# bcosm/CantorRL

Hardware: AMD Instinct MI355X
Metric: env-steps/sec (batched episodes) (higher is better)
Workload: dtype f64+f32; 1 GPU; configs[1]: 65,536 parallel envs/GPU, European call (BS rolling-ATM marks), GBM, v2 env, train_ppo_v2 reward; config_index=2, envs_per_gpu=65536, episode_length=252, mode=rollout, rollout_k=256, action_sets=1, parallelism=env-shard x1

## Files before the change

### cantorrl_amd/csrc/he_math.h

```cpp
#pragma once

#include <hip/hip_runtime.h>
#include <stdint.h>

#define HE_HD __host__ __device__ __forceinline__

namespace he {

HE_HD double fma_k(double a, double b, double c) {
#if defined(__HIP_DEVICE_COMPILE__)
    double r;
    asm("v_fma_f64 %0, %1, %2, %3" : "=v"(r) : "v"(a), "v"(b), "s"(c));
    return r;
#else
    return fma(a, b, c);
#endif
}

HE_HD double fma_kb(double a, double k, double c) {
#if defined(__HIP_DEVICE_COMPILE__)
    double r;
    asm("v_fma_f64 %0, %1, %2, %3" : "=v"(r) : "v"(a), "s"(k), "v"(c));
    return r;
#else
// ... 87 lines not shown
}

HE_HD float div_int_byf(float a, float b, float y) {
    const float q = a * y;
    return fmaf(fmaf(-q, b, a), y, q);
}
HE_HD double div_int_by(double a, double b, double y) {
    const double q = a * y;
    return fma(fma(-q, b, a), y, q);
}

HE_HD float div_f32_by(float a, double b, double y64) {
    const double ad = (double)a;
    const double q = ad * y64;
    const double r = fma(-q, b, ad);
    const float res = (float)fma(r, y64, q);
    return (a == 0.0f || !(fabsf(a) <= 3.4028234663852886e38f)) ? (float)q : res;
}

HE_HD float div_f32_byf(float a, float b, float y) {
    const float q = a * y;
    const float res = fmaf(fmaf(-q, b, a), y, q);
    return (a == 0.0f || !(fabsf(a) <= 3.4028234663852886e38f)) ? q : res;
}

HE_HD int32_t trade_round(float f, int32_t mt) {
    const float r = rintf(f);
    const bool ok = fabsf(r) < 9.2233720368547758e18f;
    const float lo = -(float)mt, hi = (float)mt;
#if defined(__HIP_DEVICE_COMPILE__)
    return ok ? (int32_t)__builtin_amdgcn_fmed3f(r, lo, hi) : -mt;
#else
    const float c = r < lo ? lo : (r > hi ? hi : r);
    const int32_t v = ok ? (int32_t)c : 0;
    return ok ? v : -mt;
#endif
}

HE_HD uint32_t episode_wrap_le(uint32_t t, uint32_t k, uint32_t T) {
    const uint32_t s = t + k;
    return s >= T ? s - T : s;
}
HE_HD uint32_t episode_wrap(uint32_t t, uint32_t k, uint32_t T) {
    return k <= T ? episode_wrap_le(t, k, T) : (t + k) % T;
}

// ... 564 lines not shown
```

### cantorrl_amd/csrc/hedge_env.hip

```cpp
#include <hip/hip_runtime.h>
#include <hip/hip_ext.h>

#include <math.h>
#include <stdarg.h>
#include <stdio.h>
#include <stdlib.h>
#include <string.h>

#include <chrono>
#include <new>
#include <type_traits>

#include "vn_moments.h"
#include <string>
#include <vector>

#include "../../include/hedge_env.h"
#include "he_math.h"

using namespace he;

namespace {

#define GLOBAL __attribute__((address_space(1)))
// ... 61 lines not shown
    float s0s_f, inv_s0s_f;
    double s0s_d, inv_s0s_d;
    double inv_252;
    float init_cash_f;
    double tcpc, slip_frac, lam, w, theta, initial_cash;
    double shares_d, inv_shares;
    float shares_f;
    int32_t shares_zero;
    float r_f, tenor_f;
    double r_d, tenor_d, sqrt_tenor;
    int32_t tenor_small;
    uint32_t key0, key1;
    double s0;
    double var;
    float var_f;
    double sqrt_var, drift, sqrt_dt, mu, dt;
    BSConst bs;
    int32_t mark;
    double fe_K;
    float g_sigma, g_num_drift;
    double g_sst;
    double g_inv_sst;
    float g_sst_f, g_inv_sst_f;
    float sqrt_tenor_f;
    double h_kappa, h_theta, h_xi, h_rho, h_sqrt1mrho2;
    int32_t den_const;
    double den, inv_den;
    int32_t M;
    float4* tileA;
    float4* tileB;
    float rstv[4 + kObs];
    const float4* rec;
    const float4* recg;
    int64_t n_paths;
    int64_t rstride;
    int32_t roff;
    int32_t book_n;
    const BookOpt* book;
    const double* book_tab;
    int32_t book_rows;
    double bk_sig, bk_isig, bk_s2, bk_lam;
    double book_rst;
    double* tileC;
#ifdef HE_TIMING
    uint64_t* tim;
#endif
// ... 122 lines not shown
            cd = (S > K) ? 1.0 : ((S == K) ? 0.5 : 0.0);
            pd = (S < K) ? -1.0 : ((S == K) ? -0.5 : 0.0);
            gam = 0.0;
        } else {
            float Kc = np_maxf(K, 1e-6f);
            float num = logf(S / Kc) + num_drift;
            double d1;
            if (sst < 1e-9) {
                float sg = (num > 0.0f) ? 1.0f : ((num < 0.0f) ? -1.0f : num);
                d1 = (double)(sg * 10.0f);
            } else {
                d1 = CONST_VAR ? (double)num * p.g_inv_sst : (double)num / sst;
            }
            double n1 = ndtr(d1);
            cd = n1;
            pd = n1 - 1.0;
            double gd = (double)S * sst;
            gam = (fabs(gd) < 1e-9) ? 0.0 : norm_pdf(d1) / gd;
        }
    }
    return make_float4((float)cd, (float)gam, (float)pd, 0.0f);
}

__device__ __forceinline__ float ncdf_tail(float d1, float ph) {
    const float a = fminf(fabsf(d1), 14.0f);
    const float w = 2.0f * __builtin_amdgcn_rcpf(a + 2.0f);
    float r = -2.690903097e-02f;
    r = fmaf(r, w, 6.361111253e-02f);
    r = fmaf(r, w, 2.313483953e-01f);
    r = fmaf(r, w, -1.219161630e+00f);
    r = fmaf(r, w, 2.182162046e+00f);
    r = fmaf(r, w, -1.785471797e+00f);
    r = fmaf(r, w, 4.304344356e-01f);
    r = fmaf(r, w, -1.690988056e-02f);
    r = fmaf(r, w, 3.958457112e-01f);
    r = fmaf(r, w, 4.983069301e-01f);
    r = fmaf(r, w, 5.000579357e-01f);
    return ph * (r * w);
}

template <bool CONST_VAR>
__device__ __forceinline__ float4 greeks_fast(const Params& p, float S, float v) {
    float cd, gam, pd;
    const float K = rintf(S);
    if (S <= 1e-6f) {
        cd = (K == 0.0f) ? 0.5f : ((K > 0.0f) ? 0.0f : 1.0f);
        pd = (K == 0.0f) ? -0.5f : ((K < 0.0f) ? 0.0f : -1.0f);
        gam = 0.0f;
// ... 28 lines not shown
            const float ph = expf(-0.5f * (d1 * d1)) * 0.398942280401432678f;
            const float tail = ncdf_tail(d1, ph);
            cd = (d1 >= 0.0f) ? 1.0f - tail : tail;
            pd = (d1 >= 0.0f) ? -tail : tail - 1.0f;
            const float gd = S * sstf;
            gam = (fabsf(gd) < 1e-9f) ? 0.0f : ph * __builtin_amdgcn_rcpf(gd);
        }
    }
    return make_float4(cd, gam, pd, 0.0f);
}

__device__ __forceinline__ float4 replay_greeks(const Params& p, float S, float v) {
    return greeks<false>(p, S, v);
}

__device__ __forceinline__ float div_f32_core(float a, float b) {
    float r = __builtin_amdgcn_rcpf(b);
    r = fmaf(fmaf(-b, r, 1.0f), r, r);
    float q = a * r;
    q = fmaf(fmaf(-b, q, a), r, q);
    return fmaf(fmaf(-b, q, a), r, q);
}

__device__ __forceinline__ float logf_normal(float x) {
    const float r = __builtin_amdgcn_logf(x);
    const float hi = r * 0x1.62e42ep-1f;
    float t = fmaf(r, 0x1.62e42ep-1f, -hi);
    t = fmaf(r, 0x1.efa39ep-25f, t);
    return (fabsf(r) < __builtin_inff()) ? hi + t : r;
}
__device__ __forceinline__ float expf_nonpos(float x) {
    const float hi = x * 0x1.715476p+0f;
    float t = fmaf(x, 0x1.715476p+0f, -hi);
    const float k = rintf(hi);
    t = fmaf(x, 0x1.4ae0bep-26f, t);
    const float e = __builtin_amdgcn_exp2f((hi - k) + t);
    const float v = ldexpf(e, (int)k);
    return (x >= -0x1.9d1da0p+6f || x != x) ? v : 0.0f;
}

__device__ __forceinline__ float4 greeks_lean(float S, float num_drift, float inv_sst_f, float sstf) {
    const float K = rintf(S);
    const float Kc = np_maxf(K, 1e-6f);
    const float num = logf_normal(div_f32_core(S, Kc)) + num_drift;
    const float d1 = num * inv_sst_f;
    const float ph = expf_nonpos(-0.5f * (d1 * d1)) * 0.398942280401432678f;
    const float tail = ncdf_tail(d1, ph);
    float cd = (d1 >= 0.0f) ? 1.0f - tail : tail;
    float pd = (d1 >= 0.0f) ? -tail : tail - 1.0f;
    const float gd = S * sstf;
    float ge = ph * __builtin_amdgcn_rcpf(gd);
    float ct = (K == 0.0f) ? 0.5f : ((K > 0.0f) ? 0.0f : 1.0f);
    float pt = (K == 0.0f) ? -0.5f : ((K < 0.0f) ? 0.0f : -1.0f);
    HE_OPAQUE3(ge, ct, pt);
    float gam = (fabsf(gd) < 1e-9f) ? 0.0f : ge;
    const bool tiny = S <= 1e-6f;
    cd = tiny ? ct : cd;
    pd = tiny ? pt : pd;
    gam = tiny ? 0.0f : gam;
    return make_float4(cd, gam, pd, 0.0f);
}

__device__ __forceinline__ int32_t clamp_pos(int32_t n, int32_t maxh) {
    int32_t r;
    asm("v_med3_i32 %0, %1, %2, %3" : "=v"(r) : "v"(n), "v"(-maxh), "v"(maxh));
    return r;
}

__device__ __forceinline__ float lag_return(float S, float Sp) {
    float q = (S - Sp) / Sp;
    HE_OPAQUE1(q);
    return (Sp == 0.0f) ? 0.0f : np_clipf(q, -1.0f, 1.0f);
}

__device__ __forceinline__ float lag_return_lean(float S, float Sp) {
    const float d = S - Sp;
    float q = div_f32_core((d > Sp) ? Sp : d, Sp);
    HE_OPAQUE1(q);
    return (Sp == 0.0f) ? 0.0f : np_clipf(q, -1.0f, 1.0f);
}

template <bool FAST = false, bool EP = false>
__device__ __forceinline__ void make_obs(const Params& p, const Env& e, const Mkt& m, float4 g, float Sp,
                                         float vp, float* o) {
    if (EP) {
        o[0] = div_f32_by(m.S, e.s0s_d, e.inv_s0s_d);
        o[1] = div_f32_by(m.C, e.s0s_d, e.inv_s0s_d);
        o[2] = div_f32_by(m.P, e.s0s_d, e.inv_s0s_d);
    } else if (FAST || p.s0s_const) {
        o[0] = div_f32_by(m.S, p.s0s_d, p.inv_s0s_d);
        o[1] = div_f32_by(m.C, p.s0s_d, p.inv_s0s_d);
        o[2] = div_f32_by(m.P, p.s0s_d, p.inv_s0s_d);
    } else {
        float s0s = np_maxf(e.s0, 25.0f);
        o[0] = m.S / s0s;
        o[1] = m.C / s0s;
        o[2] = m.P / s0s;
    }
    if (FAST || p.maxh != 0) {
// ... 1288 lines not shown
    static constexpr int prod = lanes;
    static constexpr int penvs = kLdsEnvs / lanes;
    static constexpr int threads = 64 * (2 + prod);
    static constexpr int H = kLdsM / lanes;
    static constexpr int minwaves = (BOOK || HESTON) ? kLdsMinWavesBook
                                                     : (HE_LDS_BALANCE ? 4 : (4 * (2 + prod) + 3) / 4 + 1);
    static_assert(H * lanes == kLdsM && penvs * lanes == kLdsEnvs, "producer lane layout");
};

constexpr int kLdsBookRows = 256;
constexpr int lds_thp_rows() { return 512; }
template <int MODE, bool BOOK, bool LEAN = false>
struct LdsMarketT {
    static constexpr int NB = 2;
    static constexpr bool THP = LEAN && !BOOK;
    double thp[THP ? lds_thp_rows() : 1];
    float2 sc[NB][kLdsM][kLdsEnvs];
    float pp[NB][kLdsM][kLdsEnvs];
    float stage[2][kLdsEnvs * kObs];
    double bk[BOOK ? 2 : 1][BOOK ? kLdsM : 1][kLdsEnvs];
    float vv[MODE == HE_MODE_HESTON ? 2 : 1][MODE == HE_MODE_HESTON ? kLdsM : 1][kLdsEnvs];
    double btab[BOOK ? kLdsBookRows : 1][4];
    BookOpt bopt[BOOK ? HE_BOOK_MAX : 1];
};
static_assert(kLdsM > 8 || sizeof(LdsMarketT<HE_MODE_GBM, false>) <= 40 * 1024, "4 workgroups per CU");
static_assert(kLdsM > 8 || sizeof(LdsMarketT<HE_MODE_GBM, false, true>) <= 40 * 1024 - 64, "4 workgroups per CU");
static_assert(kLdsM > 8 || sizeof(LdsMarketT<HE_MODE_HESTON, true>) <= 40 * 1024, "4 workgroups per CU");

#ifdef HE_LDS_TIMING
__device__ uint64_t g_lds_tim[4][4096][5];
#define LDS_T0() uint64_t tim_t0 = __builtin_amdgcn_s_memtime(), tim_bar = 0, tim_r0 = __builtin_amdgcn_s_memrealtime()
#define LDS_BAR()                                                  \
    do {                                                           \
        const uint64_t tb_ = __builtin_amdgcn_s_memtime();         \
        __syncthreads();                                           \
        tim_bar += __builtin_amdgcn_s_memtime() - tb_;             \
    } while (0)
#define LDS_T1(role)                                                                     \
    do {                                                                                 \
        if ((threadIdx.x & 63) == 0 && blockIdx.x < 4096) {                              \
            g_lds_tim[role][blockIdx.x][0] = __builtin_amdgcn_s_memtime() - tim_t0;      \
            g_lds_tim[role][blockIdx.x][1] = tim_bar;                                    \
            const uint64_t r1_ = __builtin_amdgcn_s_memrealtime();                       \
            g_lds_tim[role][blockIdx.x][2] = r1_ - tim_r0;                               \
            g_lds_tim[role][blockIdx.x][3] = tim_r0;                                     \
            g_lds_tim[role][blockIdx.x][4] = r1_;                                        \
        }                                                                                \
    } while (0)
#else
#define LDS_T0() do {} while (0)
#define LDS_BAR() __syncthreads()
#define LDS_T1(role) do {} while (0)
#endif

__device__ __forceinline__ void flush_obs_full(const float* img, float* out, int64_t row0, int lane) {
    asm volatile("" ::: "memory");
    GLOBAL float* dst = (GLOBAL float*)out + row0 * kObs;
    GLOBAL v4f* d4 = (GLOBAL v4f*)dst;
    const v4f* s4 = reinterpret_cast<const v4f*>(img);
    d4[lane] = s4[lane];
    d4[lane + 64] = s4[lane + 64];
    d4[lane + 128] = s4[lane + 128];
    dst[768 + lane] = img[768 + lane];
    asm volatile("" ::: "memory");
}

template <int MODE, bool BOOK, bool LEAN, bool OBS, bool POL = false, bool PLAIN_OK = false>
__device__ __forceinline__ void lds_stepper(const Params& p, State s, const Io& io, int k_steps, const Market& cur,
                                            LdsMarketT<MODE, BOOK, LEAN>& L, int64_t base) {
    constexpr int D = kLdsPrefetch;
    constexpr bool HESTON = MODE == HE_MODE_HESTON;
    const int lane = threadIdx.x & 63;
    const int64_t N = p.n;
    const int nfull = k_steps / kLdsM;
    const int tail = k_steps - nfull * kLdsM;
    const int64_t i0 = base + lane;
    const int64_t i = i0 < N ? i0 : N - 1;
    const int wrows = (int)((N - base) < kLdsEnvs ? (N - base) : kLdsEnvs);
    const Mkt rst{p.rstv[0], p.rstv[1], p.rstv[2], p.rstv[3], BOOK ? p.book_rst : 0.0};
    const GLOBAL v2f* gact = (const GLOBAL v2f*)io.act;
    GLOBAL float* const grew = (GLOBAL float*)io.rew;
    GLOBAL uint8_t* const gterm = (GLOBAL uint8_t*)io.term;
    if (!BOOK && !HESTON) {
        if (OBS) __builtin_amdgcn_s_setprio(kPrioGbmObs);
        else __builtin_amdgcn_s_setprio(kPrioGbmRew);
    } else {
        if (OBS) __builtin_amdgcn_s_setprio(kPrioObs);
        else __builtin_amdgcn_s_setprio(kPrioRewBook);
    }
    LDS_T0();
// ... 104 lines not shown
                        rec.pnl_sum = acc[1];
                        rec.abs_pnl_sum = acc[2];
                        rec.cost_sum = acc[3];
                        rec.pnl_penalty_sum = acc[4];
                        rec.cost_penalty_sum = acc[5];
                        rec.per_share_pnl_sum = acc[6];
                        rec.reserved2 = 0.0;
                        io.pol.rec[r] = rec;
                    }
                }
                last0 = (float)acc[0];
                last1 = (float)acc[1];
                last2 = (float)acc[3];
                last3 = (float)acc_len;
#pragma unroll
                for (int c = 0; c < 7; ++c) acc[c] = 0.0;
                acc_len = 0;
            }
        }
    };

    constexpr int NB = LdsMarketT<MODE, BOOK, LEAN>::NB;
    constexpr bool kPlain = PLAIN_OK && LEAN && !POL;
    auto run_blk = [&](auto&& step) {
        LDS_BAR();
        for (int b = 0; b < nfull; ++b) {
#if defined(HE_LDS_DIAG) && HE_LDS_DIAG == 2
            LDS_BAR();
            continue;
#endif
            const int buf = b % NB;
            auto slots = [&](auto plain) {
#pragma unroll
                for (int sl = 0; sl < kLdsM; ++sl) {
                    const int k = b * kLdsM + sl;
                    const float2 ak = ra[sl % D];
                    if constexpr (!POL) {
                        const int kn = k + D;
                        ra[sl % D] = ld2(gact, (int64_t)(kn < k_steps ? kn : k_steps - 1) * N + i);
                    }
                    step(buf, sl, k, ak, std::true_type{}, plain);
                }
            };
            if constexpr (kPlain) {
                if (__ballot((int32_t)(e.t + (uint32_t)kLdsM) >= p.T) == 0ull) slots(std::true_type{});
                else slots(std::false_type{});
            } else {
                slots(std::false_type{});
            }
            LDS_BAR();
        }
        if (tail) {
#if !(defined(HE_LDS_DIAG) && HE_LDS_DIAG == 2)
            const int buf = nfull % NB;
            for (int sl = 0; sl < tail; ++sl) {
                const int k = nfull * kLdsM + sl;
                step(buf, sl, k, POL ? make_float2(0.0f, 0.0f) : ld2(gact, (int64_t)k * N + i), std::false_type{},
                     std::false_type{});
            }
#endif
            LDS_BAR();
        }
    };

    if constexpr (LEAN) {
        const float mt_f = p.mt_f, maxh_f = p.maxh_f, inv_maxh_f = p.inv_maxh_f;
        const int32_t mt = p.mt, maxh = p.maxh, T = p.T;
        if (OBS) {
            const float s0s_f = p.s0s_f, inv_s0s_f = p.inv_s0s_f;
            const float T_f = p.T_f, inv_T_f = p.inv_T_f, var_f = p.var_f;
            const float gnd = p.g_num_drift, gis = p.g_inv_sst_f, gsf = p.g_sst_f;
            float ro[kObs];
#pragma unroll
            for (int c = 0; c < kObs; ++c) ro[c] = p.rstv[4 + c];
            float preS = pre.S;
            if (e.t != 0) preS = (float)cur.S[i];
            float preV = rst.v;
            if (HESTON && e.t != 0) preV = (float)cur.v[i];
            const double s0s_d = p.s0s_d, inv_s0s_d = p.inv_s0s_d;
            using lds_float = __attribute__((address_space(3))) float;
            lds_float* row0 = (lds_float*)&L.stage[0][lane * kObs];
            lds_float* row1 = (lds_float*)&L.stage[1][lane * kObs];
            asm volatile("" : "+v"(row0), "+v"(row1));
            auto obs_step = [&](int buf, int sl, int k, float2 ak, auto full, auto plain) {
                constexpr bool PLAIN = decltype(plain)::value;
                const float2 r0 = L.sc[buf][sl][lane];
                const float rP = L.pp[buf][sl][lane];
                const float vk = HESTON ? L.vv[HESTON ? buf : 0][HESTON ? sl : 0][lane] : var_f;
                float4 g;
                if constexpr (HESTON) g = greeks_fast<false>(p, r0.x, vk);
                else g = greeks_lean(r0.x, gnd, gis, gsf);
                if constexpr (POL) {
                    ak = policy_action(p, pol, e.call, e.put, po3, po4, pcd, ppd);
                    if (io.pol.act_out) {
                        v2f av = {ak.x, ak.y};
                        ((GLOBAL v2f*)io.pol.act_out)[(int64_t)k * N + i] = av;
                    }
                }
                const int32_t nc = e.call + trade_round(ak.x * mt_f, mt);
                const int32_t nq = e.put + trade_round(ak.y * mt_f, mt);
                const int32_t cc = clamp_pos(nc, maxh);
                const int32_t qq = clamp_pos(nq, maxh);
                const uint32_t t1 = e.t + 1;
                const bool term = !PLAIN && (int32_t)t1 >= T;
                float o[kObs];
                if constexpr (HESTON) {
                    o[0] = div_f32_by(r0.x, s0s_d, inv_s0s_d);
                } else {
                    o[0] = div_f32_byf(r0.x, s0s_f, inv_s0s_f);
                }
                o[1] = div_f32_by(r0.y, s0s_d, inv_s0s_d);
                o[2] = div_f32_by(rP, s0s_d, inv_s0s_d);
                o[3] = div_int_byf((float)cc, maxh_f, inv_maxh_f);
                o[4] = div_int_byf((float)qq, maxh_f, inv_maxh_f);
                o[5] = vk;
                o[6] = div_int_byf((float)(T - (int32_t)t1), T_f, inv_T_f);
                o[7] = g.x;
                o[8] = g.y;
                o[9] = g.z;
                o[10] = g.y;
                o[11] = lag_return_lean(r0.x, preS);
                o[12] = (preS == 0.0f) ? 0.0f : np_clipf(vk - (HESTON ? preV : var_f), -1.0f, 1.0f);
                float* const tile = L.stage[k & 1];
                lds_float* const row = (k & 1) ? row1 : row0;
#pragma unroll
                for (int c = 0; c < kObs; ++c) row[c] = o[c];
                if constexpr (!PLAIN) {
                    if (__ballot(term) != 0ull) {
                        if (term) {
#pragma unroll
                            for (int c = 0; c < kObs; ++c) row[c] = ro[c];
                        }
                    }
                }
                if (!POL || io.obs) {
                    float* out = io.obs + (int64_t)k * N * kObs;
                    if constexpr (decltype(full)::value) flush_obs_full(tile, out, base, lane);
                    else flush_obs_wave(tile, out, base, wrows, lane);
                }
                if constexpr (POL) {
                    po3 = term ? ro[3] : o[3];
                    po4 = term ? ro[4] : o[4];
                    pcd = term ? ro[7] : o[7];
                    ppd = term ? ro[9] : o[9];
                }
                e.t = term ? 0u : t1;
                e.call = term ? 0 : cc;
                e.put = term ? 0 : qq;
                preS = term ? rst.S : r0.x;
                if (HESTON) preV = term ? rst.v : vk;
            };
            if (wrows == kLdsEnvs)
                run_blk([&](int buf, int sl, int k, float2 ak, auto, auto plain) {
                    obs_step(buf, sl, k, ak, std::true_type{}, plain);
                });
            else
                run_blk([&](int buf, int sl, int k, float2 ak, auto, auto plain) {
                    obs_step(buf, sl, k, ak, std::false_type{}, plain);
                });
        } else {
            const double tcpc = p.tcpc, slip_frac = p.slip_frac, lam = p.lam, w = p.w, theta = p.theta;
            const double shares_d = p.shares_d, inv_shares = p.inv_shares, den = p.den, inv_den = p.inv_den;
            const double inv_252 = p.inv_252, init_cash = p.initial_cash;
            const float shares_f = p.shares_f;
            double pv0 = (double)((shares_f * rst.S + 0.0f) + p.init_cash_f);
            if (BOOK) pv0 = pv0 + rst.B;
            if constexpr (LdsMarketT<MODE, BOOK, LEAN>::THP) {
                for (int t = lane; t <= T; t += 64)
                    L.thp[t] = theta * div_int_by((double)(T - t), 252.0, inv_252);
            }
            double preC100 = (double)pre.C * 100.0, preP100 = (double)pre.P * 100.0;
            if (e.t == 0) pv_last = pv0;
            const double rstC100 = (double)rst.C * 100.0, rstP100 = (double)rst.P * 100.0;
            const float rs3 = p.rstv[4 + 3], rs4 = p.rstv[4 + 4], rs7 = p.rstv[4 + 7], rs9 = p.rstv[4 + 9];
            const float gnd = p.g_num_drift, gis = p.g_inv_sst_f, gsf = p.g_sst_f;
            run_blk([&](int buf, int sl, int k, float2 ak, auto, auto plain) {
                constexpr bool PLAIN = decltype(plain)::value;
                const int64_t koff = (int64_t)k * N;
                const float2 sc = L.sc[buf][sl][lane];
                const float pP = L.pp[buf][sl][lane];
                const double C100 = (double)sc.y * 100.0, P100 = (double)pP * 100.0;
                const double pv_prev = pv_last;
// ... 34 lines not shown
                        else g = greeks_lean(sc.x, gnd, gis, gsf);
                        gx = g.x;
                        gz = g.z;
                    }
                    po3 = term ? rs3 : div_int_byf((float)cc, maxh_f, p.inv_maxh_f);
                    po4 = term ? rs4 : div_int_byf((float)qq, maxh_f, p.inv_maxh_f);
                    pcd = term ? rs7 : gx;
                    ppd = term ? rs9 : gz;
                } else if constexpr (PLAIN) {
                    sm0 = sm0 + reward;
                    sm1 = sm1 + pnl;
                    sm2 = sm2 + tc;
                    slen = slen + 1u;
                } else {
                    account(reward, pnl, tc, term);
                }
                pv_last = term ? pv0 : pv;
                e.t = term ? 0u : t1;
                e.call = term ? 0 : cc;
                e.put = term ? 0 : qq;
                e.cash = term ? init_cash : cash;
                preC100 = term ? rstC100 : C100;
                preP100 = term ? rstP100 : P100;
            });
        }
    } else {
        if (OBS && e.t != 0) pre = Mkt{(float)cur.S[i], HESTON ? (float)cur.v[i] : p.var_f, cur.C[i], cur.P[i], 0.0};
        auto step = [&](int buf, int sl, int k, float2 ak, auto full) {
            const int64_t koff = (int64_t)k * N;
            const float2 sc = L.sc[buf][sl][lane];
            const float vk = HESTON ? L.vv[HESTON ? buf : 0][HESTON ? sl : 0][lane] : p.var_f;
            const Mkt post{sc.x, vk, sc.y, L.pp[buf][sl][lane], BOOK ? L.bk[buf][sl][lane] : 0.0};
            if constexpr (POL) ak = policy_action(p, pol, e.call, e.put, po3, po4, pcd, ppd);
            if (OBS) {
                if (POL && io.pol.act_out) {
                    v2f av = {ak.x, ak.y};
                    ((GLOBAL v2f*)io.pol.act_out)[koff + i] = av;
                }
                float4 g = p.record_metrics ? greeks_fast<!HESTON>(p, post.S, post.v) : make_float4(0.f, 0.f, 0.f, 0.f);
                g.w = lag_return(post.S, pre.S);
                const int32_t nc = e.call + trade_round(ak.x * p.mt_f, p.mt);
                const int32_t nq = e.put + trade_round(ak.y * p.mt_f, p.mt);
                e.call = clamp_pos(nc, p.maxh);
                e.put = clamp_pos(nq, p.maxh);
                e.t = e.t + 1;
                const bool term = (int32_t)e.t >= p.T;
                float o[kObs];
// ... 19 lines not shown
                pv_last = so.pv;
                if (grew) grew[koff + i] = (float)so.reward;
                if (gterm) gterm[koff + i] = so.term ? 1 : 0;
                if constexpr (POL) {
                    pol_account(so.reward, so.pnl, so.ps, so.tc, so.rpc, so.tcp, so.term);
                    float gx = 0.0f, gz = 0.0f;
                    if (pol_greeks && prm) {
                        const float4 g = greeks_fast<!HESTON>(p, post.S, post.v);
                        gx = g.x;
                        gz = g.z;
                    }
                    po3 = so.term ? p.rstv[4 + 3] : (pmh ? div_int_byf((float)e.call, p.maxh_f, p.inv_maxh_f) : 0.0f);
                    po4 = so.term ? p.rstv[4 + 4] : (pmh ? div_int_byf((float)e.put, p.maxh_f, p.inv_maxh_f) : 0.0f);
                    pcd = so.term ? p.rstv[4 + 7] : gx;
                    ppd = so.term ? p.rstv[4 + 9] : gz;
                } else {
                    account(so.reward, so.pnl, so.tc, so.term);
                }
                pre = so.term ? rst : post;
                if (so.term) env_reset_common(p, e);
            }
        };
        if (OBS && wrows == kLdsEnvs)
            run_blk([&](int buf, int sl, int k, float2 ak, auto, auto) { step(buf, sl, k, ak, std::true_type{}); });
        else
            run_blk([&](int buf, int sl, int k, float2 ak, auto, auto) { step(buf, sl, k, ak, std::false_type{}); });
    }
    LDS_T1(OBS ? 1 : 0);
    if (!OBS && i0 < N) {
        int64_t j = i;
        asm volatile("" : "+v"(j));
        s.t[j] = e.t;
        s.pos[j] = pack_pos(e.call, e.put);
        s.cash[j] = e.cash;
        if constexpr (POL) {
#pragma unroll
            for (int c = 0; c < 7; ++c) s.acc[(int64_t)c * N + j] = acc[c];
            s.acc_len[j] = acc_len;
        } else {
            s.sum[j] = sm0;
            s.sum[N + j] = sm1;
            s.sum[2 * N + j] = sm2;
            s.sum_len[j] = slen;
        }
        s.last[j] = last0;
        s.last[N + j] = last1;
        s.last[2 * N + j] = last2;
        s.last[3 * N + j] = last3;
    }
}

__device__ __forceinline__ void prod_prio_toggle(bool up) {
    if (up) __builtin_amdgcn_s_setprio(kPrioProd + 1);
    else __builtin_amdgcn_s_setprio(kPrioProd);
}

template <int MODE, bool BOOK, bool LEAN, bool PLAIN_OK = false>
__device__ __forceinline__ void lds_producer(const Params& p, int k_steps, const Market& cur,
                                             LdsMarketT<MODE, BOOK, LEAN>& W, int64_t base, int pw) {
    using G = LdsGeom<MODE, BOOK>;
    constexpr bool HESTON = G::HESTON;
    constexpr int kLdsLanes = G::lanes, kLdsPEnvs = G::penvs, kLdsH = G::H;
    const int lane = threadIdx.x & 63;
    const int sub = lane / kLdsPEnvs;
    const int le = pw * kLdsPEnvs + (lane % kLdsPEnvs);
    const int64_t N = p.n;
    const int nb = (k_steps + kLdsM - 1) / kLdsM;
    const uint32_t T = (uint32_t)p.T;
    const int64_t pi = (base + le) < N ? base + le : N - 1;
    if (!BOOK && !HESTON) {
        if (pw == 0) __builtin_amdgcn_s_setprio(kPrioGbmProd0);
        else __builtin_amdgcn_s_setprio(kPrioGbmProd1);
    } else {
        __builtin_amdgcn_s_setprio(kPrioProd);
    }
    uint64_t a0;
    uint32_t tpb;
    {
        const uint32_t ep0 = cur.ep[pi], t0 = cur.t[pi];
        const uint32_t off = t0 >= T ? T : t0;
        a0 = (uint64_t)ep0 * T + off;
        tpb = off >= T ? 0u : off;
    }
    double Sbs = cur.S[pi];
    double Vbs = HESTON ? cur.v[pi] : 0.0;
    double Mbs = BOOK ? cur.M[pi] : 0.0;
    const int sl0 = sub * kLdsH;
    LDS_T0();
    for (int bp = 0; bp <= nb; ++bp) {
#if defined(HE_LDS_DIAG) && HE_LDS_DIAG == 1
        LDS_BAR();
        continue;
#endif
        if (bp < nb) {
            const int kb = bp * kLdsM;
            const int len = (k_steps - kb) < kLdsM ? (k_steps - kb) : kLdsM;
            auto block = [&](auto full, auto plain) {
                constexpr bool FULL = decltype(full)::value;
                constexpr bool PLAIN = decltype(plain)::value;
                constexpr bool LOCK = FULL && LEAN && !HESTON;

            const int64_t gid = p.goff + pi;
            const uint64_t nf = a0 + (uint64_t)(kb + sl0);
            const uint32_t tpf = PLAIN ? 0u : episode_wrap(tpb, (uint32_t)sl0, T);
            double ex[kLdsH];
            double Vx[kLdsH];
            double Vin = Vbs;
            if constexpr (LOCK) {
                const uint64_t m0 = nf >> 1;
                const bool odd = (nf & 1) != 0;
// ... 91 lines not shown
                        sqx[h] = (j == sl0 + h) ? sq : sqx[h];
                        Vx[h] = (j == sl0 + h) ? v : Vx[h];
                    }
                }
                Vbs = v;
#pragma unroll
                for (int h = 0; h < kLdsH; ++h) {
                    const double drift = (p.mu - 0.5 * vpx[h]) * p.dt;
                    const double diff = sqx[h] * ws[h];
                    ex[h] = (FULL || sl0 + h < len) ? exp(drift + diff) : 1.0;
                }
            }
            double eall[kLdsM];
#pragma unroll
            for (int r = 0; r < kLdsLanes; ++r)
#pragma unroll
                for (int h = 0; h < kLdsH; ++h) eall[r * kLdsH + h] = __shfl(ex[h], (lane % kLdsPEnvs) + r * kLdsPEnvs);
            double Sx[kLdsH], Mx[kLdsH];
#pragma unroll
            for (int h = 0; h < kLdsH; ++h) Sx[h] = Sbs;
#pragma unroll
            for (int h = 0; h < kLdsH; ++h) Mx[h] = Mbs;
            double S = Sbs, Sin = Sbs, Mr = Mbs;
            {
                uint32_t tp = tpb;
#pragma unroll
                for (int j = 0; j < kLdsM; ++j) {
                    if (j == sl0) Sin = S;
                    if (FULL || j < len) {
                        if (!PLAIN && tp == 0) {
                            S = p.s0;
                            if (BOOK) Mr = p.s0;
                        }
                        const double Sn = S * eall[j];
                        S = (Sn < 1e-8) ? 1e-8 : Sn;
                        if (BOOK) Mr = np_max(Mr, S);
                        if (!PLAIN) tp = (tp + 1 == T) ? 0u : tp + 1;
                    }
#pragma unroll
                    for (int h = 0; h < kLdsH; ++h) Sx[h] = (j == sl0 + h) ? S : Sx[h];
                    if (BOOK) {
#pragma unroll
                        for (int h = 0; h < kLdsH; ++h) Mx[h] = (j == sl0 + h) ? Mr : Mx[h];
                    }
                }
            }
            Sbs = S;
            if (BOOK) Mbs = Mr;
            uint32_t tp = tpf;
            const int wb = bp % LdsMarketT<MODE, BOOK, LEAN>::NB;
            double lkC[kLdsH], lkP[kLdsH];
            if constexpr (LOCK) {
                double Sm[kLdsH], Km[kLdsH];
                uint32_t tq = tpf;
#pragma unroll
                for (int h = 0; h < kLdsH; ++h) {
                    if constexpr (PLAIN) {
                        Sm[h] = Sx[h];
                    } else {
                        const bool last = tq + 1 == T;
                        const double Sprev = (h == 0) ? Sin : Sx[h - 1];
                        Sm[h] = last ? ((tq == 0) ? p.s0 : Sprev) : Sx[h];
                        tq = (tq + 1 == T) ? 0u : tq + 1;
                    }
                    Km[h] = rint(Sm[h]);
                }
                bs_call_put_n<kLdsH>(Sm, Km, p.bs, lkC, lkP);
            }
            if constexpr (LOCK) {
#pragma unroll
                for (int h = 0; h < kLdsH; ++h) {
                    const int sl = sl0 + h;
                    W.sc[wb][sl][le] = make_float2((float)Sx[h], (float)lkC[h]);
                    W.pp[wb][sl][le] = (float)lkP[h];
                }
            } else {
                double rS[kLdsH], rV[kLdsH];
#pragma unroll
                for (int h = 0; h < kLdsH; ++h) {
                    rS[h] = Sx[h];
                    rV[h] = HESTON ? Vx[h] : p.var;
                }
                double Sprev = Sin, Vprev = Vin;
#pragma unroll 1
                for (int h = 0; h < kLdsH; ++h) {
                    if (FULL || sl0 + h < len) {
                        const bool last = tp + 1 == T;
                        const double Sm = last ? ((tp == 0) ? p.s0 : Sprev) : rS[0];
                        const double Vh = rV[0];
                        const double Vm = HESTON ? (last ? ((tp == 0) ? p.var : Vprev) : Vh) : p.var;
// ... 111 lines not shown
    }
#endif
    return wave;
}

constexpr int kLdsNumSgpr = 96;
constexpr bool kPlainPersistS = false, kPlainPersistP = true;
template <int MODE, bool BOOK, bool LEAN, bool PERSIST = false, bool POL = false>
__global__ __launch_bounds__((LdsGeom<MODE, BOOK>::threads), (LdsGeom<MODE, BOOK>::minwaves))
    __attribute__((amdgpu_num_sgpr(kLdsNumSgpr))) void lds_rollout_kernel(const Params* __restrict__ pc, State s, Io io,
                                                                 int k_steps, Market cur) {
    __shared__ __attribute__((aligned(16))) LdsMarketT<MODE, BOOK, LEAN> lm;
    const Params& p = *pc;
    const int wave = lds_role<LdsGeom<MODE, BOOK>::threads / 64>(__builtin_amdgcn_readfirstlane(threadIdx.x >> 6));
    if constexpr (BOOK) {
        const int nv = 4 * p.book_rows;
        for (int k = threadIdx.x; k < nv; k += LdsGeom<MODE, BOOK>::threads) (&lm.btab[0][0])[k] = p.book_tab[k];
        if ((int)threadIdx.x < p.book_n) lm.bopt[threadIdx.x] = p.book[threadIdx.x];
        __syncthreads();
    }
    if constexpr (!PERSIST) {
        const int64_t base = (int64_t)blockIdx.x * kLdsEnvs;
        if (wave == 0) lds_stepper<MODE, BOOK, LEAN, false, POL, true>(p, s, io, k_steps, cur, lm, base);
        else if (wave == 1) lds_stepper<MODE, BOOK, LEAN, true, POL, true>(p, s, io, k_steps, cur, lm, base);
        else lds_producer<MODE, BOOK, LEAN, true>(p, k_steps, cur, lm, base, wave - 2);
        return;
    }
    const int64_t tiles = (p.n + kLdsEnvs - 1) / kLdsEnvs;
    for (int64_t tile = blockIdx.x; tile < tiles; tile += gridDim.x) {
        asm volatile("" ::: "memory");
        const int64_t base = tile * kLdsEnvs;
        if (wave == 0) lds_stepper<MODE, BOOK, LEAN, false, POL, kPlainPersistS>(p, s, io, k_steps, cur, lm, base);
        else if (wave == 1) lds_stepper<MODE, BOOK, LEAN, true, POL, kPlainPersistS>(p, s, io, k_steps, cur, lm, base);
        else lds_producer<MODE, BOOK, LEAN, kPlainPersistP>(p, k_steps, cur, lm, base, wave - 2);
        if (tile + gridDim.x < tiles) __syncthreads();
    }
}

struct LdsReplay {
    float4 mk[2][kLdsM][kLdsEnvs];
    float2 gd[2][kLdsM][kLdsEnvs];
    float gg[2][kLdsM][kLdsEnvs];
    float4 rk[2][kLdsEnvs];
    float4 rg[2][kLdsEnvs];
    float stage[2][kLdsEnvs * kObs];
};
static_assert(kLdsM > 8 || sizeof(LdsReplay) <= 40 * 1024 - 64, "4 workgroups per CU");

// ... 745 lines not shown
static he_status fail(he_env* env, he_status st, const char* fmt, ...) {
    char buf[512];
    va_list ap;
    va_start(ap, fmt);
    vsnprintf(buf, sizeof(buf), fmt, ap);
    va_end(ap);
    if (env) env->err = buf;
    return st;
}

#define HE_HIP(env, call)                                                                      \
    do {                                                                                       \
        hipError_t _e = (call);                                                                \
        if (_e != hipSuccess)                                                                  \
            return fail((env), HE_EHIP, "%s failed: %s", #call, hipGetErrorString(_e));        \
    } while (0)

static bool is_generate(const he_env* env) { return env->cfg.mode != HE_MODE_REPLAY; }

#ifdef HE_TIMING
static uint64_t* g_tim = nullptr;
#endif

static void fill_params(he_env* env) {
    const he_config& c = env->cfg;
    Params& p = env->p;
    memset(&p, 0, sizeof(p));
    p.n = c.n_envs;
    p.goff = c.global_env_offset;
    p.variant = c.variant;
    p.loss = c.loss_type;
    p.record_metrics = c.record_metrics ? 1 : 0;
    {
        const char* ev = getenv("HE_GREEKS_IN_STEP_MIN_ENVS");
        const int64_t thr = (ev && *ev) ? (int64_t)atoll(ev) : kGreeksInStepMinEnvs;
        p.tile_greeks = (c.mode == HE_MODE_HESTON || c.n_envs < thr) ? 1 : 0;
    }
    p.autoreset = c.autoreset ? 1 : 0;
    p.mode = c.mode;
    p.mt = c.max_trade_per_step;
    p.maxh = c.max_contracts_held_per_type;
    p.mt_f = (float)c.max_trade_per_step;
    p.maxh_f = (float)c.max_contracts_held_per_type;
    p.init_cash_f = (float)c.initial_cash;
    p.tcpc = c.transaction_cost_per_contract;
    p.slip_frac = c.slippage_bps / 10000.0;
// ... 18 lines not shown
    p.var_f = (float)c.variance;
    p.mu = c.mu;
    p.dt = c.dt;
    p.sqrt_dt = sqrt(c.dt);
    p.drift = (c.mu - 0.5 * c.variance) * c.dt;
    p.sqrt_var = sqrt(c.variance < 0.0 ? 0.0 : c.variance);
    double sig = sqrt(c.variance < 0.0 ? 0.0 : c.variance);
    double T = c.option_tenor_years, r = c.risk_free_rate;
    p.bs.intrinsic = (T <= 0.0) || (sig <= 0.0);
    p.bs.a = (r + 0.5 * pow(sig, 2.0)) * T;
    p.bs.b = sig * sqrt(T);
    p.bs.inv_b = 1.0 / p.bs.b;
    p.bs.disc = exp(-r * T);
    p.mark = c.mark;
    p.fe_K = rint(c.s0);
    float vf = (float)c.variance;
    float vmax = (vf != vf) ? vf : (vf > 1e-8f ? vf : 1e-8f);
    p.g_sigma = sqrtf(vmax);
    p.g_num_drift = ((float)r + 0.5f * powf(p.g_sigma, 2.0f)) * (float)T;
    p.g_sst = (double)p.g_sigma * sqrt(T);
    p.g_inv_sst = 1.0 / p.g_sst;
    p.g_sst_f = (float)p.g_sst;
    p.g_inv_sst_f = (float)p.g_inv_sst;
    p.sqrt_tenor_f = (float)p.sqrt_tenor;
    p.h_kappa = c.heston_kappa;
    p.h_theta = c.heston_theta;
    p.h_xi = c.heston_xi;
    p.h_rho = c.heston_rho;
    double omr = 1.0 - c.heston_rho * c.heston_rho;
    p.h_sqrt1mrho2 = sqrt(omr < 0.0 ? 0.0 : omr);
    p.T = c.episode_length;
    p.T_f = (float)c.episode_length;
    p.inv_maxh_f = 1.0f / p.maxh_f;
    p.inv_T_f = 1.0f / p.T_f;
    p.inv_252 = 1.0 / 252.0;
    p.M = c.market_block;
    p.tileA = p.tileB = nullptr;
    memcpy(p.rstv, env->rstv, sizeof(p.rstv));
    if (is_generate(env)) {
        float s0 = p.rstv[0];
        bool small = s0 < 1e-6f;
        float f = small ? 25.0f : (s0 > 25.0f || s0 != s0 ? s0 : 25.0f);
        if (c.loss_type == HE_LOSS_MSE) p.den = small ? (625.0 + 1e-9) : (double)(f * f + 1e-9f);
        else p.den = small ? (25.0 + 1e-9) : (double)(f + 1e-9f);
        p.inv_den = 1.0 / p.den;
        p.den_const = 1;
// ... 1329 lines not shown
```

Measured before the change: 64.14 billion env-steps/s.

## Add range-checked fast path that drops edge-case guards in GBM obs step

The producer waves now compute a per-block verdict from the exponent bits of prices and marks, checking that all values lie in a safe range, and publish it to LDS. A host-side check on the parameters sets a flag when d1 stays bounded. When both hold for the whole wave, the stepper runs a 'tame' variant that skips the clamps, NaN/inf guards, tiny-S branches and zero checks in greeks, logf/expf, division and lag-return. The change also precomputes the constant GBM variance delta observation. This trims ALU work in the hot observation loop, at the cost of extra producer reductions, LDS traffic and a ballot per block.

New measurement: 67.48 billion env-steps/s, median of 6. 5.2% higher.

```diff
diff --git a/cantorrl_amd/csrc/he_math.h b/cantorrl_amd/csrc/he_math.h
--- a/cantorrl_amd/csrc/he_math.h
+++ b/cantorrl_amd/csrc/he_math.h
@@ -133,6 +133,16 @@
     const float q = a * y;
     const float res = fmaf(fmaf(-q, b, a), y, q);
     return (a == 0.0f || !(fabsf(a) <= 3.4028234663852886e38f)) ? q : res;
+}
+
+HE_HD float div_f32_by_nz(float a, double b, double y64) {
+    const double ad = (double)a;
+    const double q = ad * y64;
+    return (float)fma(fma(-q, b, ad), y64, q);
+}
+HE_HD float div_f32_byf_nz(float a, float b, float y) {
+    const float q = a * y;
+    return fmaf(fmaf(-q, b, a), y, q);
 }
 
 HE_HD int32_t trade_round(float f, int32_t mt) {
diff --git a/cantorrl_amd/csrc/hedge_env.hip b/cantorrl_amd/csrc/hedge_env.hip
--- a/cantorrl_amd/csrc/hedge_env.hip
+++ b/cantorrl_amd/csrc/hedge_env.hip
@@ -107,6 +107,7 @@
     double g_sst;
     double g_inv_sst;
     float g_sst_f, g_inv_sst_f;
+    int32_t lds_tame;
     float sqrt_tenor_f;
     double h_kappa, h_theta, h_xi, h_rho, h_sqrt1mrho2;
     int32_t den_const;
@@ -275,8 +276,9 @@
     return make_float4((float)cd, (float)gam, (float)pd, 0.0f);
 }
 
+template <bool TAME = false>
 __device__ __forceinline__ float ncdf_tail(float d1, float ph) {
-    const float a = fminf(fabsf(d1), 14.0f);
+    const float a = TAME ? fabsf(d1) : fminf(fabsf(d1), 14.0f);
     const float w = 2.0f * __builtin_amdgcn_rcpf(a + 2.0f);
     float r = -2.690903097e-02f;
     r = fmaf(r, w, 6.361111253e-02f);
@@ -351,13 +353,16 @@
     return fmaf(fmaf(-b, q, a), r, q);
 }
 
+template <bool FINITE = false>
 __device__ __forceinline__ float logf_normal(float x) {
     const float r = __builtin_amdgcn_logf(x);
     const float hi = r * 0x1.62e42ep-1f;
     float t = fmaf(r, 0x1.62e42ep-1f, -hi);
     t = fmaf(r, 0x1.efa39ep-25f, t);
+    if constexpr (FINITE) return hi + t;
     return (fabsf(r) < __builtin_inff()) ? hi + t : r;
 }
+template <bool INRANGE = false>
 __device__ __forceinline__ float expf_nonpos(float x) {
     const float hi = x * 0x1.715476p+0f;
     float t = fmaf(x, 0x1.715476p+0f, -hi);
@@ -365,10 +370,25 @@
     t = fmaf(x, 0x1.4ae0bep-26f, t);
     const float e = __builtin_amdgcn_exp2f((hi - k) + t);
     const float v = ldexpf(e, (int)k);
+    if constexpr (INRANGE) return v;
     return (x >= -0x1.9d1da0p+6f || x != x) ? v : 0.0f;
 }
 
-__device__ __forceinline__ float4 greeks_lean(float S, float num_drift, float inv_sst_f, float sstf) {
+template <bool TAME>
+__device__ __forceinline__ float4 greeks_lean_t(float S, float num_drift, float inv_sst_f, float sstf) {
+    const float K = rintf(S);
+    const float num = logf_normal<true>(div_f32_core(S, K)) + num_drift;
+    const float d1 = num * inv_sst_f;
+    const float ph = expf_nonpos<true>(-0.5f * (d1 * d1)) * 0.398942280401432678f;
+    const float tail = ncdf_tail<true>(d1, ph);
+    const float cd = (d1 >= 0.0f) ? 1.0f - tail : tail;
+    const float pd = (d1 >= 0.0f) ? -tail : tail - 1.0f;
+    const float gd = S * sstf;
+    const float gam = ph * __builtin_amdgcn_rcpf(gd);
+    return make_float4(cd, gam, pd, 0.0f);
+}
+template <>
+__device__ __forceinline__ float4 greeks_lean_t<false>(float S, float num_drift, float inv_sst_f, float sstf) {
     const float K = rintf(S);
     const float Kc = np_maxf(K, 1e-6f);
     const float num = logf_normal(div_f32_core(S, Kc)) + num_drift;
@@ -389,6 +409,9 @@
     gam = tiny ? 0.0f : gam;
     return make_float4(cd, gam, pd, 0.0f);
 }
+__device__ __forceinline__ float4 greeks_lean(float S, float num_drift, float inv_sst_f, float sstf) {
+    return greeks_lean_t<false>(S, num_drift, inv_sst_f, sstf);
+}
 
 __device__ __forceinline__ int32_t clamp_pos(int32_t n, int32_t maxh) {
     int32_t r;
@@ -402,8 +425,13 @@
     return (Sp == 0.0f) ? 0.0f : np_clipf(q, -1.0f, 1.0f);
 }
 
+template <bool TAME = false>
 __device__ __forceinline__ float lag_return_lean(float S, float Sp) {
     const float d = S - Sp;
+    if constexpr (TAME) {
+        const float q = div_f32_core((d > Sp) ? Sp : d, Sp);
+        return __builtin_amdgcn_fmed3f(q, -1.0f, 1.0f);
+    }
     float q = div_f32_core((d > Sp) ? Sp : d, Sp);
     HE_OPAQUE1(q);
     return (Sp == 0.0f) ? 0.0f : np_clipf(q, -1.0f, 1.0f);
@@ -1738,6 +1766,7 @@
     float vv[MODE == HE_MODE_HESTON ? 2 : 1][MODE == HE_MODE_HESTON ? kLdsM : 1][kLdsEnvs];
     double btab[BOOK ? kLdsBookRows : 1][4];
     BookOpt bopt[BOOK ? HE_BOOK_MAX : 1];
+    uint32_t tame[NB][2];
 };
 static_assert(kLdsM > 8 || sizeof(LdsMarketT<HE_MODE_GBM, false>) <= 40 * 1024, "4 workgroups per CU");
 static_assert(kLdsM > 8 || sizeof(LdsMarketT<HE_MODE_GBM, false, true>) <= 40 * 1024 - 64, "4 workgroups per CU");
@@ -1781,7 +1810,7 @@
     asm volatile("" ::: "memory");
 }
 
-template <int MODE, bool BOOK, bool LEAN, bool OBS, bool POL = false, bool PLAIN_OK = false>
+template <int MODE, bool BOOK, bool LEAN, bool OBS, bool POL = false, bool PLAIN_OK = false, bool TAME_OK = false>
 __device__ __forceinline__ void lds_stepper(const Params& p, State s, const Io& io, int k_steps, const Market& cur,
                                             LdsMarketT<MODE, BOOK, LEAN>& L, int64_t base) {
     constexpr int D = kLdsPrefetch;
@@ -1932,7 +1961,9 @@
 
     constexpr int NB = LdsMarketT<MODE, BOOK, LEAN>::NB;
     constexpr bool kPlain = PLAIN_OK && LEAN && !POL;
-    auto run_blk = [&](auto&& step) {
+    constexpr bool kTame = kPlain && TAME_OK && OBS && MODE == HE_MODE_GBM && !BOOK;
+    const bool tame_h = kTame && p.lds_tame != 0;
+    auto run_blk = [&](auto&& step, auto&& pre_ok) {
         LDS_BAR();
         for (int b = 0; b < nfull; ++b) {
 #if defined(HE_LDS_DIAG) && HE_LDS_DIAG == 2
@@ -1953,8 +1984,17 @@
                 }
             };
             if constexpr (kPlain) {
-                if (__ballot((int32_t)(e.t + (uint32_t)kLdsM) >= p.T) == 0ull) slots(std::true_type{});
-                else slots(std::false_type{});
+                if (__ballot((int32_t)(e.t + (uint32_t)kLdsM) >= p.T) == 0ull) {
+                    if constexpr (kTame) {
+                        const uint32_t tw = __builtin_amdgcn_readfirstlane(L.tame[buf][0] & L.tame[buf][1]);
+                        if (tame_h && tw != 0u && __ballot(!pre_ok()) == 0ull) slots(std::integral_constant<int, 2>{});
+                        else slots(std::true_type{});
+                    } else {
+                        slots(std::true_type{});
+                    }
+                } else {
+                    slots(std::false_type{});
+                }
             } else {
                 slots(std::false_type{});
             }
@@ -1985,6 +2025,8 @@
             for (int c = 0; c < kObs; ++c) ro[c] = p.rstv[4 + c];
             float preS = pre.S;
             if (e.t != 0) preS = (float)cur.S[i];
+            const float dv12 = np_clipf(var_f - var_f, -1.0f, 1.0f);
+            auto pre_ok = [&] { return preS >= 64.0f && preS <= 8388608.0f; };
             float preV = rst.v;
             if (HESTON && e.t != 0) preV = (float)cur.v[i];
             const double s0s_d = p.s0s_d, inv_s0s_d = p.inv_s0s_d;
@@ -1994,12 +2036,13 @@
             asm volatile("" : "+v"(row0), "+v"(row1));
             auto obs_step = [&](int buf, int sl, int k, float2 ak, auto full, auto plain) {
                 constexpr bool PLAIN = decltype(plain)::value;
+                constexpr bool TAME = (int)decltype(plain)::value == 2;
                 const float2 r0 = L.sc[buf][sl][lane];
                 const float rP = L.pp[buf][sl][lane];
                 const float vk = HESTON ? L.vv[HESTON ? buf : 0][HESTON ? sl : 0][lane] : var_f;
                 float4 g;
                 if constexpr (HESTON) g = greeks_fast<false>(p, r0.x, vk);
-                else g = greeks_lean(r0.x, gnd, gis, gsf);
+                else g = greeks_lean_t<TAME>(r0.x, gnd, gis, gsf);
                 if constexpr (POL) {
                     ak = policy_action(p, pol, e.call, e.put, po3, po4, pcd, ppd);
                     if (io.pol.act_out) {
@@ -2014,13 +2057,19 @@
                 const uint32_t t1 = e.t + 1;
                 const bool term = !PLAIN && (int32_t)t1 >= T;
                 float o[kObs];
-                if constexpr (HESTON) {
-                    o[0] = div_f32_by(r0.x, s0s_d, inv_s0s_d);
+                if constexpr (TAME) {
+                    o[0] = div_f32_byf_nz(r0.x, s0s_f, inv_s0s_f);
+                    o[1] = div_f32_by_nz(r0.y, s0s_d, inv_s0s_d);
+                    o[2] = div_f32_by_nz(rP, s0s_d, inv_s0s_d);
                 } else {
-                    o[0] = div_f32_byf(r0.x, s0s_f, inv_s0s_f);
+                    if constexpr (HESTON) {
+                        o[0] = div_f32_by(r0.x, s0s_d, inv_s0s_d);
+                    } else {
+                        o[0] = div_f32_byf(r0.x, s0s_f, inv_s0s_f);
+                    }
+                    o[1] = div_f32_by(r0.y, s0s_d, inv_s0s_d);
+                    o[2] = div_f32_by(rP, s0s_d, inv_s0s_d);
                 }
-                o[1] = div_f32_by(r0.y, s0s_d, inv_s0s_d);
-                o[2] = div_f32_by(rP, s0s_d, inv_s0s_d);
                 o[3] = div_int_byf((float)cc, maxh_f, inv_maxh_f);
                 o[4] = div_int_byf((float)qq, maxh_f, inv_maxh_f);
                 o[5] = vk;
@@ -2029,8 +2078,10 @@
                 o[8] = g.y;
                 o[9] = g.z;
                 o[10] = g.y;
-                o[11] = lag_return_lean(r0.x, preS);
-                o[12] = (preS == 0.0f) ? 0.0f : np_clipf(vk - (HESTON ? preV : var_f), -1.0f, 1.0f);
+                o[11] = lag_return_lean<TAME>(r0.x, preS);
+                if constexpr (HESTON) o[12] = (preS == 0.0f) ? 0.0f : np_clipf(vk - preV, -1.0f, 1.0f);
+                else if constexpr (TAME) o[12] = 0.0f;
+                else o[12] = (preS == 0.0f) ? 0.0f : dv12;
                 float* const tile = L.stage[k & 1];
                 lds_float* const row = (k & 1) ? row1 : row0;
 #pragma unroll
@@ -2063,11 +2114,11 @@
             if (wrows == kLdsEnvs)
                 run_blk([&](int buf, int sl, int k, float2 ak, auto, auto plain) {
                     obs_step(buf, sl, k, ak, std::true_type{}, plain);
-                });
+                }, pre_ok);
             else
                 run_blk([&](int buf, int sl, int k, float2 ak, auto, auto plain) {
                     obs_step(buf, sl, k, ak, std::false_type{}, plain);
-                });
+                }, pre_ok);
         } else {
             const double tcpc = p.tcpc, slip_frac = p.slip_frac, lam = p.lam, w = p.w, theta = p.theta;
             const double shares_d = p.shares_d, inv_shares = p.inv_shares, den = p.den, inv_den = p.inv_den;
@@ -2148,7 +2199,7 @@
                 e.cash = term ? init_cash : cash;
                 preC100 = term ? rstC100 : C100;
                 preP100 = term ? rstP100 : P100;
-            });
+            }, [] { return false; });
         }
     } else {
         if (OBS && e.t != 0) pre = Mkt{(float)cur.S[i], HESTON ? (float)cur.v[i] : p.var_f, cur.C[i], cur.P[i], 0.0};
@@ -2214,9 +2265,11 @@
             }
         };
         if (OBS && wrows == kLdsEnvs)
-            run_blk([&](int buf, int sl, int k, float2 ak, auto, auto) { step(buf, sl, k, ak, std::true_type{}); });
+            run_blk([&](int buf, int sl, int k, float2 ak, auto, auto) { step(buf, sl, k, ak, std::true_type{}); },
+                    [] { return false; });
         else
-            run_blk([&](int buf, int sl, int k, float2 ak, auto, auto) { step(buf, sl, k, ak, std::false_type{}); });
+            run_blk([&](int buf, int sl, int k, float2 ak, auto, auto) { step(buf, sl, k, ak, std::false_type{}); },
+                    [] { return false; });
     }
     LDS_T1(OBS ? 1 : 0);
     if (!OBS && i0 < N) {
@@ -2247,7 +2300,7 @@
     else __builtin_amdgcn_s_setprio(kPrioProd);
 }
 
-template <int MODE, bool BOOK, bool LEAN, bool PLAIN_OK = false>
+template <int MODE, bool BOOK, bool LEAN, bool PLAIN_OK = false, bool TAME_OK = false>
 __device__ __forceinline__ void lds_producer(const Params& p, int k_steps, const Market& cur,
                                              LdsMarketT<MODE, BOOK, LEAN>& W, int64_t base, int pw) {
     using G = LdsGeom<MODE, BOOK>;
@@ -2278,6 +2331,7 @@
     double Vbs = HESTON ? cur.v[pi] : 0.0;
     double Mbs = BOOK ? cur.M[pi] : 0.0;
     const int sl0 = sub * kLdsH;
+    constexpr bool kTame = TAME_OK && PLAIN_OK && LEAN && !HESTON && !BOOK && kLdsLanes == 2;
     LDS_T0();
     for (int bp = 0; bp <= nb; ++bp) {
 #if defined(HE_LDS_DIAG) && HE_LDS_DIAG == 1
@@ -2415,7 +2469,23 @@
 #pragma unroll
             for (int h = 0; h < kLdsH; ++h) Mx[h] = Mbs;
             double S = Sbs, Sin = Sbs, Mr = Mbs;
-            {
+            if constexpr (kTame && FULL) {
+                static_assert(!kTame || kLdsM == 2 * kLdsH, "two lanes per env");
+                double Sa[kLdsM];
+                uint32_t tp = tpb;
+#pragma unroll
+                for (int j = 0; j < kLdsM; ++j) {
+                    if (!PLAIN && tp == 0) S = p.s0;
+                    const double Sn = S * eall[j];
+                    S = (Sn < 1e-8) ? 1e-8 : Sn;
+                    if (!PLAIN) tp = (tp + 1 == T) ? 0u : tp + 1;
+                    Sa[j] = S;
+                }
+                const bool hi = sub != 0;
+#pragma unroll
+                for (int h = 0; h < kLdsH; ++h) Sx[h] = hi ? Sa[kLdsH + h] : Sa[h];
+                Sin = hi ? Sa[kLdsH - 1] : Sbs;
+            } else {
                 uint32_t tp = tpb;
 #pragma unroll
                 for (int j = 0; j < kLdsM; ++j) {
@@ -2459,6 +2529,27 @@
                     Km[h] = rint(Sm[h]);
                 }
                 bs_call_put_n<kLdsH>(Sm, Km, p.bs, lkC, lkP);
+            }
+            if constexpr (kTame) {
+                uint32_t verdict = 0u;
+                if constexpr (LOCK && PLAIN) {
+                    uint32_t smin = (uint32_t)__double2hiint(Sx[0]), smax = smin;
+                    uint32_t mmin = (uint32_t)__double2hiint(lkC[0]), mmax = mmin;
+#pragma unroll
+                    for (int h = 0; h < kLdsH; ++h) {
+                        const uint32_t sh = (uint32_t)__double2hiint(Sx[h]);
+                        const uint32_t ch = (uint32_t)__double2hiint(lkC[h]), ph = (uint32_t)__double2hiint(lkP[h]);
+                        smin = sh < smin ? sh : smin;
+                        smax = sh > smax ? sh : smax;
+                        mmin = ch < mmin ? ch : mmin;
+                        mmax = ch > mmax ? ch : mmax;
+                        mmin = ph < mmin ? ph : mmin;
+                        mmax = ph > mmax ? ph : mmax;
+                    }
+                    const bool ok = smin >= 0x40500000u && smax < 0x41600000u && mmin >= 0x38100000u && mmax < 0x47e00000u;
+                    verdict = __ballot(!ok) == 0ull ? 0xffffffffu : 0u;
+                }
+                W.tame[wb][pw] = verdict;
             }
             if constexpr (LOCK) {
 #pragma unroll
@@ -2616,8 +2707,8 @@
     if constexpr (!PERSIST) {
         const int64_t base = (int64_t)blockIdx.x * kLdsEnvs;
         if (wave == 0) lds_stepper<MODE, BOOK, LEAN, false, POL, true>(p, s, io, k_steps, cur, lm, base);
-        else if (wave == 1) lds_stepper<MODE, BOOK, LEAN, true, POL, true>(p, s, io, k_steps, cur, lm, base);
-        else lds_producer<MODE, BOOK, LEAN, true>(p, k_steps, cur, lm, base, wave - 2);
+        else if (wave == 1) lds_stepper<MODE, BOOK, LEAN, true, POL, true, !POL>(p, s, io, k_steps, cur, lm, base);
+        else lds_producer<MODE, BOOK, LEAN, true, !POL>(p, k_steps, cur, lm, base, wave - 2);
         return;
     }
     const int64_t tiles = (p.n + kLdsEnvs - 1) / kLdsEnvs;
@@ -3409,6 +3500,12 @@
 static uint64_t* g_tim = nullptr;
 #endif
 
+static bool lds_tame_handle(const Params& p) {
+    const double d1_max = (0.008 + fabs((double)p.g_num_drift)) * fabs((double)p.g_inv_sst_f) * (1.0 + 1e-5);
+    return d1_max < 14.0 && p.g_inv_sst_f > 0.0f && 64.0f * p.g_sst_f >= 1e-9f && 64.0f * p.g_sst_f < 3.0e38f &&
+           fabsf(p.var_f) <= 3.4028234663852886e38f;
+}
+
 static void fill_params(he_env* env) {
     const he_config& c = env->cfg;
     Params& p = env->p;
@@ -3473,6 +3570,7 @@
     p.g_inv_sst = 1.0 / p.g_sst;
     p.g_sst_f = (float)p.g_sst;
     p.g_inv_sst_f = (float)p.g_inv_sst;
+    p.lds_tame = lds_tame_handle(p) ? 1 : 0;
     p.sqrt_tenor_f = (float)p.sqrt_tenor;
     p.h_kappa = c.heston_kappa;
     p.h_theta = c.heston_theta;
```
